# tbennun/capital

Measured on NVIDIA H100. Metric: cholesky_tflops_fp64, higher is better.
Workload: dtype f64

## Files before the change

### capital_b200/csrc/leaf.cu

```cuda
#include "common.cuh"
#include "tile64.cuh"
#include <cooperative_groups.h>
#include <cfloat>
#include <stdlib.h>
#include <type_traits>
namespace cg = cooperative_groups;

namespace {
constexpr int LD = LEAF_MAX + 1;

__device__ __forceinline__ double fast_rsqrt(double d) {
  if (!(d > 1e-30 && d < 1e30)) return rsqrt(d);
  double y = (double)rsqrtf((float)d);
  const double h = 0.5 * d;
  y = y * fma(-h, y * y, 1.5);
  y = y * fma(-h, y * y, 1.5);
  return y;
}

__device__ void leaf_factor_invert(int nb, double* __restrict__ a, double* __restrict__ r, double* __restrict__ t, int* info,
                                   int pivot_base) {
  const int tid = threadIdx.x, tx = tid & 15, ty = tid >> 4;
  for (int k = 0; k < nb; k++) {
    if (tid < 64 && tid >= k && tid < nb) {
      double d = a[k + k * LD];
      if (!(d > 0.0)) {
        if (tid == k) atomicCAS(info, 0, pivot_base + k + 1);
        d = 1.0;
      }
      const double rs = rsqrt(d);
      r[k + tid * LD] = (tid == k) ? d * rs : a[k + tid * LD] * rs;
    }
    __syncthreads();
#pragma unroll
    for (int ia = 0; ia < 4; ia++) {
      const int i = ty + 16 * ia;
      if (i > k && i < nb) {
        const double ri = r[k + i * LD];
#pragma unroll
        for (int jb = 0; jb < 4; jb++) {
          const int j = tx + 16 * jb;
          if (j >= i && j < nb) a[i + j * LD] -= ri * r[k + j * LD];
        }
      }
    }
    __syncthreads();
  }
#pragma unroll
  for (int ia = 0; ia < 4; ia++) {
    const int i = ty + 16 * ia;
#pragma unroll
    for (int jb = 0; jb < 4; jb++) {
      const int j = tx + 16 * jb;
      if (i < nb && j < nb) {
        if (i > j) r[i + j * LD] = 0.0;
        a[i + j * LD] = (i == j) ? 1.0 / r[i + i * LD] : 0.0;
      }
    }
  }
  __syncthreads();
  int lg = 0;
  for (int bs = 1; bs < nb; bs <<= 1, lg++) {
    const int span = 2 * bs;
    const int npairs = (nb + span - 1) / span;
    const int per = bs * bs, total = npairs * per;
    for (int idx = tid; idx < total; idx += 256) {
      const int p = idx >> (2 * lg), e = idx & (per - 1);
      const int li = e & (bs - 1), lj = e >> lg;
      const int o = p * span, i = o + li, j = o + bs + lj;
      if (j < nb) {
        double s = 0.0;
        const int kend = o + bs;
        for (int k = i; k < kend; k++) s += a[i + k * LD] * r[k + j * LD];
        t[i + j * LD] = s;
      }
    }
    __syncthreads();
    for (int idx = tid; idx < total; idx += 256) {
      const int p = idx >> (2 * lg), e = idx & (per - 1);
      const int li = e & (bs - 1), lj = e >> lg;
      const int o = p * span, i = o + li, j = o + bs + lj;
      if (j < nb) {
        double s = 0.0;
        for (int k = o + bs; k <= j; k++) s += t[i + k * LD] * a[k + j * LD];
        a[i + j * LD] = -s;
      }
    }
    __syncthreads();
  }
}

__device__ __forceinline__ void leaf_load(int nb, const double* W, long long ldw, double* __restrict__ a) {
  for (int idx = threadIdx.x; idx < nb * nb; idx += 256) {
    const int i = idx % nb, j = idx / nb;
    a[i + j * LD] = (i <= j) ? __ldcg(W + i + (long long)j * ldw) : 0.0;
  }
}
__device__ __forceinline__ void leaf_store(int nb, const double* a, const double* r, double* __restrict__ R,
                                           long long ldr, double* __restrict__ Ri, long long ldri, double* __restrict__ RiT,
                                           long long ldrit) {
  for (int idx = threadIdx.x; idx < nb * nb; idx += 256) {
    const int i = idx % nb, j = idx / nb;
    R[i + (long long)j * ldr] = r[i + j * LD];
    Ri[i + (long long)j * ldri] = a[i + j * LD];
  }
  if (RiT != nullptr) {
    for (int idx = threadIdx.x; idx < nb * nb; idx += 256) {
      const int j = idx % nb, i = idx / nb;
      RiT[j + (long long)i * ldrit] = a[i + j * LD];
    }
  }
}

__global__ void __launch_bounds__(256, 1)
    leaf_kernel(int nb, const double* W, long long ldw, double* __restrict__ R, long long ldr, double* __restrict__ Ri,
                long long ldri, double* __restrict__ RiT, long long ldrit, int* __restrict__ info, BatchStrides bs,
                int pivot_base) {
  extern __shared__ double sm[];
  double* a = sm;
  double* r = sm + LEAF_MAX * LD;
  double* t = sm + 2 * LEAF_MAX * LD;
  const long long b = blockIdx.x;
  W += b * bs.w; R += b * bs.r; Ri += b * bs.ri; info += b;
  if (RiT != nullptr) RiT += b * bs.rit;
  leaf_load(nb, W, ldw, a);
  __syncthreads();
  leaf_factor_invert(nb, a, r, t, info, pivot_base);
  leaf_store(nb, a, r, R, ldr, Ri, ldri, RiT, ldrit);
}

template <bool ACCUM>
__device__ __forceinline__ void tile_store(double* __restrict__ dst, long long ld, const double* sC) {
  const int r2 = (threadIdx.x & 31) * 2, c0 = threadIdx.x >> 5;
#pragma unroll
  for (int r = 0; r < 8; r++) {
    const int c = c0 + 8 * r;
    double2 v = *reinterpret_cast<const double2*>(sC + c * TLD + r2);
    double2* p = reinterpret_cast<double2*>(dst + r2 + (long long)c * ld);
    if (ACCUM) { const double2 o = __ldcg(p); v.x += o.x; v.y += o.y; }
    *p = v;
  }
}
__device__ __forceinline__ void tile_store_from_rowmajor(double* __restrict__ dst, long long ld, const double* sCr) {
  const int c2 = (threadIdx.x & 31) * 2, r0 = threadIdx.x >> 5;
#pragma unroll
  for (int r = 0; r < 8; r++) {
    const int row = r0 + 8 * r;
    const double2 v = *reinterpret_cast<const double2*>(sCr + row * TLD + c2);
    *reinterpret_cast<double2*>(dst + c2 + (long long)row * ld) = v;
  }
}

__device__ __forceinline__ double shfl_d(double v, int src) { return __shfl_sync(0xffffffffu, v, src); }

template <int I, int END, int STEP = 1, typename F>
__device__ __forceinline__ void static_for(F&& f) {
  if constexpr (I < END) {
    f(std::integral_constant<int, I>{});
    static_for<I + STEP, END, STEP>(f);
  }
}

__device__ __forceinline__ void warp_potrf_trtri_32(double (&c)[32], double* __restrict__ sRb, double* __restrict__ sXb, double* __restrict__ sXTb,
                                                    double* __restrict__ ub, int lane, int* info, int pivot_base, long long* dbg2) {
  double myrs = 0.0;
  if (dbg2 && lane == 0) dbg2[0] = clock64();
  double dl = 0.0;
  static_for<0, 32>([&](auto ic) { constexpr int i = decltype(ic)::value; if (lane == i) dl = c[i]; });
  const bool equil = !__all_sync(0xffffffffu, dl >= 0x1p-400 && dl <= 0x1p400);
  double fl = 1.0;
  if (equil) {
    if (dl > 0.0 && dl <= DBL_MAX) fl = ldexp(1.0, -(ilogb(dl) >> 1));
    static_for<0, 32>([&](auto ic) { constexpr int i = decltype(ic)::value; c[i] = c[i] * shfl_d(fl, i) * fl; });
  }
  double a = shfl_d(c[0], 0), l = shfl_d(c[0], 1), b = shfl_d(c[1], 1);
  static_for<0, 32, 2>([&](auto kc) {
    constexpr int k = decltype(kc)::value;
    if (!(a > 0.0)) { if (lane == k) atomicCAS(info, 0, pivot_base + k + 1); a = 1.0; }
    double det = fma(b, a, -(l * l));
    if (!(det > 0.0)) { if (lane == k + 1) atomicCAS(info, 0, pivot_base + k + 2); det = 1.0; }
    const double ra = fast_rsqrt(a), rdet = fast_rsqrt(det);
    const double sa = a * ra, lk = l * ra, rs2 = sa * rdet;
    const double u0 = (lane > k) ? c[k] * ra : (lane == k ? sa : 0.0);
    const double t1 = fma(-lk, u0, c[k + 1]);
    const double u1 = (lane > k + 1) ? t1 * rs2 : (lane == k + 1 ? det * rdet * ra : 0.0);
    c[k] = u0;
    c[k + 1] = u1;
    if (lane == k) myrs = ra;
    if (lane == k + 1) myrs = rs2;
    double* row0 = ub + (k & 2) * 32;
    double* row1 = row0 + 32;
    row0[lane] = u0;
    row1[lane] = u1;
    __syncwarp();
    if constexpr (k + 2 < 32) {
      c[k + 2] = fma(-row1[k + 2], u1, fma(-row0[k + 2], u0, c[k + 2]));
      c[k + 3] = fma(-row1[k + 3], u1, fma(-row0[k + 3], u0, c[k + 3]));
      a = shfl_d(c[k + 2], k + 2);
      l = shfl_d(c[k + 2], k + 3);
      b = shfl_d(c[k + 3], k + 3);
      static_for<k + 4, 32>([&](auto ic) {
        constexpr int i = decltype(ic)::value;
        c[i] = fma(-row1[i], u1, fma(-row0[i], u0, c[i]));
      });
    }
  });
  if (equil) {
    const double gl = 1.0 / fl;
    static_for<0, 32>([&](auto ic) { constexpr int i = decltype(ic)::value; c[i] *= gl; });
    myrs *= fl;
  }
  if (dbg2 && lane == 0) dbg2[1] = clock64();
#pragma unroll
  for (int i = 0; i < 32; i++) sRb[lane * TLD + i] = c[i];
  __syncwarp();
  const int g16 = lane >> 4, jl = lane & 15, base = 16 * g16;
  double xl[16];
  static_for<0, 16>([&](auto rc_) { constexpr int r = decltype(rc_)::value; xl[r] = (r == jl) ? myrs : 0.0; });
  static_for<0, 15>([&](auto sc) {
    constexpr int il = 14 - decltype(sc)::value;
    const double rsi = shfl_d(myrs, base + il);
    double s0 = 0.0, s1 = 0.0, s2 = 0.0, s3 = 0.0;
    static_for<il + 1, 16>([&](auto tc) {
      constexpr int t = decltype(tc)::value;
      const double rit = sRb[(base + t) * TLD + base + il];
      if constexpr ((t & 3) == 0) s0 = fma(rit, xl[t], s0);
      else if constexpr ((t & 3) == 1) s1 = fma(rit, xl[t], s1);
      else if constexpr ((t & 3) == 2) s2 = fma(rit, xl[t], s2);
      else s3 = fma(rit, xl[t], s3);
    });
    if (jl > il) xl[il] = -rsi * ((s0 + s1) + (s2 + s3));
  });
  double* xs = ub + 128;
  double* ts = ub + 128 + 512;
  static_for<0, 16>([&](auto rc_) {
    constexpr int r = decltype(rc_)::value;
    xs[lane * 16 + r] = xl[r];
    sXb[lane * TLD + base + r] = xl[r];
    sXTb[(base + r) * TLD + lane] = xl[r];
  });
  __syncwarp();
  {
    double rc[16], tr[8];
    static_for<0, 16>([&](auto tc) { constexpr int t = decltype(tc)::value; rc[t] = sRb[(16 + jl) * TLD + t]; });
    static_for<0, 8>([&](auto rr) {
      constexpr int r = decltype(rr)::value;
      const int i = 8 * g16 + r;
      double s = 0.0;
      static_for<0, 16>([&](auto tc) {
        constexpr int t = decltype(tc)::value;
        s = fma(xs[t * 16 + i], rc[t], s);
      });
      tr[r] = s;
      ts[jl * 16 + i] = s;
    });
    __syncwarp();
    double xc[16];
    static_for<0, 16>([&](auto tc) { constexpr int t = decltype(tc)::value; xc[t] = xs[(16 + jl) * 16 + t]; });
    static_for<0, 8>([&](auto rr) {
      constexpr int r = decltype(rr)::value;
      const int i = 8 * g16 + r;
      double s = 0.0;
      static_for<0, 16>([&](auto tc) {
        constexpr int t = decltype(tc)::value;
        s = fma(ts[t * 16 + i], xc[t], s);
      });
      sXb[(16 + jl) * TLD + i] = -s;
      sXTb[i * TLD + 16 + jl] = -s;
    });
    (void)tr;
  }
  __syncwarp();
  if (dbg2 && lane == 0) dbg2[2] = clock64();
}

__device__ __forceinline__ void mma32(double (&acc)[2][2], const double* As, int ar, const double* Bs, int bc, int k0) {
  const int lane = threadIdx.x & 31, w = threadIdx.x >> 5, g = lane >> 2, q = lane & 3;
  const double* ap = As + (ar + (w & 3) * 8 + g) * TLD + k0 + q;
  const double* bp = Bs + (bc + (w >> 2) * 16 + g) * TLD + k0 + q;
#pragma unroll
  for (int k = 0; k < 32; k += 4) {
    const double a = ap[k], b0 = bp[k], b1 = bp[8 * TLD + k];
    dmma884(acc[0][0], acc[0][1], a, b0);
    dmma884(acc[1][0], acc[1][1], a, b1);
  }
}
#define M32_ROW ((w & 3) * 8 + g)
#define M32_COL(j, e) ((w >> 2) * 16 + (j) * 8 + 2 * q + (e))

__device__ void leaf64_fast(double* __restrict__ sA, double* __restrict__ sR, double* __restrict__ sX, double* __restrict__ sXT,
                            double* __restrict__ ub, int* info, int pivot_base, long long* dbg2 = nullptr) {
  const int tid = threadIdx.x, lane = tid & 31, w = tid >> 5, g = lane >> 2, q = lane & 3;
  for (int idx = tid; idx < 64 * 64; idx += 256) {
    const int r = idx & 63, cidx = idx >> 6;
    sR[cidx * TLD + r] = 0.0; sX[cidx * TLD + r] = 0.0; sXT[cidx * TLD + r] = 0.0;
  }
  __syncthreads();
  double c[32];
#pragma unroll 1
  for (int half = 0; half < 2; half++) {
    const int o = half * 32;
    if (half == 1) {
      double acc[2][2] = {{0.0, 0.0}, {0.0, 0.0}};
      mma32(acc, sX, 0, sA, 32, 0);
#pragma unroll
      for (int j = 0; j < 2; j++)
#pragma unroll
        for (int e = 0; e < 2; e++) sR[(32 + M32_COL(j, e)) * TLD + M32_ROW] = acc[j][e];
      __syncthreads();
      double acc2[2][2] = {{0.0, 0.0}, {0.0, 0.0}};
      mma32(acc2, sR + 32 * TLD, 0, sR + 32 * TLD, 0, 0);
#pragma unroll
      for (int j = 0; j < 2; j++)
#pragma unroll
        for (int e = 0; e < 2; e++) sA[(32 + M32_COL(j, e)) * TLD + 32 + M32_ROW] -= acc2[j][e];
      __syncthreads();
    }
    if (w == 0) {
#pragma unroll
      for (int i = 0; i < 32; i++) c[i] = sA[(o + lane) * TLD + o + i];
      warp_potrf_trtri_32(c, sR + o * TLD + o, sX + o * TLD + o, sXT + o * TLD + o, ub, lane, info, pivot_base + o,
                          (dbg2 && half == 0) ? dbg2 : nullptr);
      if (dbg2 && half == 0 && lane == 0) dbg2[3] = clock64();
    }
    __syncthreads();
  }
  {
    double acc[2][2] = {{0.0, 0.0}, {0.0, 0.0}};
    mma32(acc, sXT, 0, sR, 32, 0);
    __syncthreads();
#pragma unroll
    for (int j = 0; j < 2; j++)
#pragma unroll
      for (int e = 0; e < 2; e++) sA[M32_ROW * TLD + 32 + M32_COL(j, e)] = acc[j][e];
    __syncthreads();
    double acc2[2][2] = {{0.0, 0.0}, {0.0, 0.0}};
    mma32(acc2, sA, 0, sX, 32, 32);
#pragma unroll
    for (int j = 0; j < 2; j++)
#pragma unroll
      for (int e = 0; e < 2; e++) {
        const double v = -acc2[j][e];
        sX[(32 + M32_COL(j, e)) * TLD + M32_ROW] = v;
        sXT[M32_ROW * TLD + 32 + M32_COL(j, e)] = v;
      }
  }
  __syncthreads();
}

template <int CW>
__global__ void __cluster_dims__(CW, 1, 1) __launch_bounds__(256, 1)
    basecase_kernel(int nb, double* __restrict__ W, long long ldw, double* __restrict__ R, long long ldr, double* __restrict__ Ri,
                    long long ldri, double* __restrict__ RiT, long long ldrit, int* __restrict__ info, long long* __restrict__ dbg,
                    BatchStrides bstr, int pivot_base) {
  {
    const long long b = blockIdx.y;
    W += b * bstr.w; R += b * bstr.r; Ri += b * bstr.ri; RiT += b * bstr.rit; info += b;
  }
  extern __shared__ __align__(16) double sm[];
  double* sA = sm;
  double* sB = sm + TILE_DOUBLES;
  double* sT = sm + 2 * TILE_DOUBLES;
  cg::cluster_group cluster = cg::this_cluster();
  const int rank = (int)cluster.block_rank();
  const int T = nb >> 6;
  double acc[4][2][2];
  int dbgi = 0;
#define DBG_STAMP() do { if (dbg && rank == 0 && threadIdx.x == 0) dbg[dbgi++] = clock64(); } while (0)
  DBG_STAMP();

  double* sU = sm + 3 * TILE_DOUBLES;
  auto do_leaf = [&](int jb) {
    const long long o = (long long)jb * 64;
    __syncthreads();
    tile_load(sA, W + o + o * ldw, ldw);
    __syncthreads();
    if (dbg && jb == 0 && threadIdx.x == 0) dbg[20] = clock64();
    leaf64_fast(sA, sB, sT, sU, sm + 4 * TILE_DOUBLES, info, pivot_base + jb * 64, (dbg && jb == 0) ? dbg + 24 : nullptr);
    if (dbg && jb == 0 && threadIdx.x == 0) dbg[21] = clock64();
    tile_store<false>(R + o + o * ldr, ldr, sB);
    tile_store<false>(Ri + o + o * ldri, ldri, sT);
    tile_store<false>(RiT + o + o * ldrit, ldrit, sU);
    __syncthreads();
  };
  auto do_trailing = [&](int jb, int i, int j) {
    const long long o = (long long)jb * 64;
    __syncthreads();
    tile_load(sA, R + o + (long long)i * 64 * ldr, ldr);
    tile_load(sB, R + o + (long long)j * 64 * ldr, ldr);
    __syncthreads();
    acc_zero(acc);
    tile_mma(acc, sA, sB);
    acc_to_smem_colmajor(acc, sT, -1.0);
    __syncthreads();
    tile_store<true>(W + (long long)i * 64 + (long long)j * 64 * ldw, ldw, sT);
  };

  if (rank == 0) do_leaf(0);
  DBG_STAMP();
  __threadfence();
  cluster.sync();
  DBG_STAMP();
  for (int jb = 0; jb < T; jb++) {
    const long long o = (long long)jb * 64;
    int work = 0;
    for (int j = jb + 1; j < T; j++, work++) {
      if (work % CW != rank) continue;
      __syncthreads();
      tile_load(sA, Ri + o + o * ldri, ldri);
      tile_load(sB, W + o + (long long)j * 64 * ldw, ldw);
      __syncthreads();
      acc_zero(acc);
      tile_mma(acc, sA, sB);
      acc_to_smem_colmajor(acc, sT, 1.0);
      __syncthreads();
      tile_store<false>(R + o + (long long)j * 64 * ldr, ldr, sT);
    }
    if (jb == 0) DBG_STAMP();
    __threadfence();
    cluster.sync();
    if (jb == 0) DBG_STAMP();
    if (jb + 1 < T) {
      const int leaf_rank = (jb + 1) % CW;
      if (rank == leaf_rank) {
        do_trailing(jb, jb + 1, jb + 1);
        __threadfence_block();
        do_leaf(jb + 1);
      } else {
        const int slot = rank > leaf_rank ? rank - 1 : rank;
        work = 0;
        for (int j = jb + 1; j < T; j++)
          for (int i = jb + 1; i <= j; i++) {
            if (i == jb + 1 && j == jb + 1) continue;
            if (work++ % (CW - 1) != slot) continue;
            do_trailing(jb, i, j);
          }
      }
    }
    if (jb == 0) DBG_STAMP();
    __threadfence();
    cluster.sync();
    if (jb == 0) DBG_STAMP();
  }
  DBG_STAMP();
  {
    int work = 0;
    for (int j = 0; j < T; j++)
      for (int i = j + 1; i < T; i++, work++) {
        if (work % CW != rank) continue;
        for (int idx = threadIdx.x; idx < 4096; idx += 256)
          R[(long long)i * 64 + (idx & 63) + ((long long)j * 64 + (idx >> 6)) * ldr] = 0.0;
      }
  }
  for (int bs = 1; bs < T; bs <<= 1) {
    const int span = 2 * bs;
    int work = 0;
    for (int o = 0; o + bs < T; o += span) {
      const int jend = min(o + span, T);
      for (int j = o + bs; j < jend; j++)
        for (int i = o; i < o + bs; i++, work++) {
          if (work % CW != rank) continue;
          acc_zero(acc);
          for (int k = i; k < o + bs; k++) {
            __syncthreads();
            tile_load(sA, RiT + (long long)k * 64 + (long long)i * 64 * ldrit, ldrit);
            tile_load(sB, R + (long long)k * 64 + (long long)j * 64 * ldr, ldr);
            __syncthreads();
            tile_mma(acc, sA, sB);
          }
          __syncthreads();
          acc_to_smem_rowmajor(acc, sT, 1.0);
          __syncthreads();
          tile_store_from_rowmajor(W + (long long)j * 64 + (long long)i * 64 * ldw, ldw, sT);
        }
    }
    __threadfence();
    cluster.sync();
    work = 0;
    for (int o = 0; o + bs < T; o += span) {
      const int jend = min(o + span, T);
      for (int j = o + bs; j < jend; j++)
        for (int i = o; i < o + bs; i++, work++) {
          if (work % CW != rank) continue;
          acc_zero(acc);
          for (int k = o + bs; k <= j; k++) {
            __syncthreads();
            tile_load(sA, W + (long long)k * 64 + (long long)i * 64 * ldw, ldw);
            tile_load(sB, Ri + (long long)k * 64 + (long long)j * 64 * ldri, ldri);
            __syncthreads();
            tile_mma(acc, sA, sB);
          }
          __syncthreads();
          acc_to_smem_colmajor(acc, sA, -1.0);
          acc_to_smem_rowmajor(acc, sB, -1.0);
          __syncthreads();
          tile_store<false>(Ri + (long long)i * 64 + (long long)j * 64 * ldri, ldri, sA);
          tile_store_from_rowmajor(RiT + (long long)j * 64 + (long long)i * 64 * ldrit, ldrit, sB);
        }
    }
    __threadfence();
    cluster.sync();
  }
  DBG_STAMP();
}
}

namespace {
constexpr int LEAF_SMEM = 3 * LEAF_MAX * LD * (int)sizeof(double);
constexpr int BASECASE_SMEM = (4 * TILE_DOUBLES + 128 + 512 + 256) * (int)sizeof(double);
}
capital_status_t leaf_init(capital_ctx* ctx) {
  CAP_CUDA(cudaFuncSetAttribute(leaf_kernel, cudaFuncAttributeMaxDynamicSharedMemorySize, LEAF_SMEM));
  CAP_CUDA(cudaFuncSetAttribute(basecase_kernel<2>, cudaFuncAttributeMaxDynamicSharedMemorySize, BASECASE_SMEM));
  CAP_CUDA(cudaFuncSetAttribute(basecase_kernel<4>, cudaFuncAttributeMaxDynamicSharedMemorySize, BASECASE_SMEM));
  CAP_CUDA(cudaFuncSetAttribute(basecase_kernel<8>, cudaFuncAttributeMaxDynamicSharedMemorySize, BASECASE_SMEM));
  return CAPITAL_OK;
}

capital_status_t leaf_cholinv(capital_ctx* ctx, cudaStream_t st, int nb, const double* W, int64_t ldw, double* R, int64_t ldr, double* Ri,
                              int64_t ldri, double* RiT, int64_t ldrit, const LeafBatch* bt, int pivot_base) {
  if (nb <= 0) return CAPITAL_OK;
  if (nb > LEAF_MAX || (bt && (bt->batch < 1 || bt->batch > INT32_MAX))) return CAPITAL_ERR_INVALID;
  constexpr int smem = LEAF_SMEM;
  const int tli = ctx->tl_begin(st, 4, nb);
  leaf_kernel<<<bt ? (unsigned)bt->batch : 1u, 256, smem, st>>>(nb, W, ldw, R, ldr, Ri, ldri, RiT, ldrit, bt ? bt->info : ctx->d_info,
                                                                bt ? bt->s : BatchStrides{}, pivot_base);
  ctx->tl_end(st, tli);
  ctx->counters.kernel_launches++;
  ctx->counters.leaf_launches++;
  CAP_CUDA(cudaGetLastError());
  return CAPITAL_OK;
}

capital_status_t basecase_cholinv(capital_ctx* ctx, cudaStream_t st, int nb, double* W, int64_t ldw, double* R, int64_t ldr, double* Ri,
                                  int64_t ldri, double* RiT, int64_t ldrit, const LeafBatch* bt, int pivot_base) {
  if (nb % 64 != 0 || nb < 64 || nb > BASECASE_MAX || RiT == nullptr) return CAPITAL_ERR_INVALID;
  const int cw = bt ? bt->cw : 8;
  if (bt && (bt->batch < 1 || bt->batch > 65535)) return CAPITAL_ERR_INVALID;
  auto kernel = cw == 2 ? basecase_kernel<2> : cw == 4 ? basecase_kernel<4> : cw == 8 ? basecase_kernel<8> : nullptr;
  if (!kernel) return CAPITAL_ERR_INVALID;
  constexpr int smem = BASECASE_SMEM;
  long long* dbg = nullptr;
  if (getenv("CAPITAL_BC_DEBUG") && !bt) {
    CAP_TRY(ctx->workspace("bc_dbg", 64 * sizeof(long long), (void**)&dbg));
    CAP_CUDA(cudaMemsetAsync(dbg, 0, 64 * sizeof(long long), st));
  }
  const int tli = ctx->tl_begin(st, 3, nb);
  kernel<<<dim3(cw, bt ? (unsigned)bt->batch : 1u), 256, smem, st>>>(nb, W, ldw, R, ldr, Ri, ldri, RiT, ldrit, bt ? bt->info : ctx->d_info,
                                                                      dbg, bt ? bt->s : BatchStrides{}, pivot_base);
  ctx->tl_end(st, tli);
  if (dbg) {
    long long h[32];
    CAP_CUDA(cudaMemcpyAsync(h, dbg, sizeof(h), cudaMemcpyDeviceToHost, st));
    CAP_CUDA(cudaStreamSynchronize(st));
    fprintf(stderr, "[bc nb=%d] leaf0=%lld bar=%lld panel0=%lld bar=%lld trail0+leaf1=%lld bar=%lld | chol_total=%lld inverse=%lld total=%lld cycles\n", nb,
            h[1] - h[0], h[2] - h[1], h[3] - h[2], h[4] - h[3], h[5] - h[4], h[6] - h[5], h[7] - h[0], h[8] - h[7], h[8] - h[0]);
    fprintf(stderr, "   leaf64: load=%lld total=%lld | warp32: pre=%lld potrf=%lld trtri=%lld store=%lld\n", h[20] - h[0], h[21] - h[20], h[24] - h[20],
            h[25] - h[24], h[26] - h[25], h[27] - h[26]);
  }
  ctx->counters.kernel_launches++;
  ctx->counters.leaf_launches++;
  CAP_CUDA(cudaGetLastError());
  return CAPITAL_OK;
}
```

### capital_b200/csrc/tile64.cuh

```cuda
#pragma once
#include "common.cuh"

namespace {
constexpr int TLD = 68;
constexpr int TILE_DOUBLES = 64 * TLD;

__device__ __forceinline__ void dmma884(double& c0, double& c1, double a, double b) {
  asm("mma.sync.aligned.m8n8k4.row.col.f64.f64.f64.f64 {%0,%1}, {%2}, {%3}, {%0,%1};" : "+d"(c0), "+d"(c1) : "d"(a), "d"(b));
}
__device__ __forceinline__ void tile_load(double* __restrict__ dst, const double* src, long long ld) {
  const int k2 = (threadIdx.x & 31) * 2, c0 = threadIdx.x >> 5;
  double2 v[8];
#pragma unroll
  for (int r = 0; r < 8; r++) v[r] = __ldcg(reinterpret_cast<const double2*>(src + k2 + (long long)(c0 + 8 * r) * ld));
#pragma unroll
  for (int r = 0; r < 8; r++) *reinterpret_cast<double2*>(dst + (c0 + 8 * r) * TLD + k2) = v[r];
}
__device__ __forceinline__ void tile_mma(double (&acc)[4][2][2], const double* As, const double* Bs) {
  const int lane = threadIdx.x & 31, w = threadIdx.x >> 5, g = lane >> 2, q = lane & 3;
  const double* ap = As + ((w & 1) * 32 + g) * TLD + q;
  const double* bp = Bs + ((w >> 1) * 16 + g) * TLD + q;
#pragma unroll 4
  for (int k0 = 0; k0 < 64; k0 += 4) {
    double af[4], bf[2];
#pragma unroll
    for (int i = 0; i < 4; i++) af[i] = ap[i * 8 * TLD + k0];
#pragma unroll
    for (int j = 0; j < 2; j++) bf[j] = bp[j * 8 * TLD + k0];
#pragma unroll
    for (int i = 0; i < 4; i++)
#pragma unroll
      for (int j = 0; j < 2; j++) dmma884(acc[i][j][0], acc[i][j][1], af[i], bf[j]);
  }
}
__device__ __forceinline__ void acc_zero(double (&acc)[4][2][2]) {
#pragma unroll
  for (int i = 0; i < 4; i++)
#pragma unroll
    for (int j = 0; j < 2; j++) acc[i][j][0] = acc[i][j][1] = 0.0;
}
#define TILE_ROW(i) ((w & 1) * 32 + (i) * 8 + g)
#define TILE_COL(j, e) ((w >> 1) * 16 + (j) * 8 + 2 * q + (e))
__device__ __forceinline__ void acc_to_smem_colmajor(const double (&acc)[4][2][2], double* __restrict__ sC, double scale) {
  const int lane = threadIdx.x & 31, w = threadIdx.x >> 5, g = lane >> 2, q = lane & 3;
#pragma unroll
  for (int i = 0; i < 4; i++)
#pragma unroll
    for (int j = 0; j < 2; j++)
#pragma unroll
      for (int e = 0; e < 2; e++) sC[TILE_COL(j, e) * TLD + TILE_ROW(i)] = scale * acc[i][j][e];
}
__device__ __forceinline__ void acc_to_smem_rowmajor(const double (&acc)[4][2][2], double* __restrict__ sC, double scale) {
  const int lane = threadIdx.x & 31, w = threadIdx.x >> 5, g = lane >> 2, q = lane & 3;
#pragma unroll
  for (int i = 0; i < 4; i++)
#pragma unroll
    for (int j = 0; j < 2; j++)
#pragma unroll
      for (int e = 0; e < 2; e++) sC[TILE_ROW(i) * TLD + TILE_COL(j, e)] = scale * acc[i][j][e];
}
}
```

Measured before the change: 33.46.

## Pipeline cluster basecase with split arrive/wait barriers and overlapped inversion

Restructures the clustered basecase kernel so rank 0 runs the critical-path leaf factorizations while the other ranks handle panels, trailing updates and triangular-inverse tiles. Full cluster.sync calls are replaced by split barrier.cluster arrive/wait, and leaf input is kept resident in shared memory. A precomputed schedule lets inverse tiles run early, interleaved with the factorization. K-loops in the inverse use double-buffered cp.async. This is meant to cut barrier stalls and serialization on the leaf critical path, at the cost of much more complex scheduling and a greater risk of ordering bugs.

```diff
diff --git a/capital_b200/csrc/leaf.cu b/capital_b200/csrc/leaf.cu
--- a/capital_b200/csrc/leaf.cu
+++ b/capital_b200/csrc/leaf.cu
@@ -348,6 +348,13 @@
   __syncthreads();
 }
 
+__device__ __forceinline__ void cluster_arrive() { asm volatile("barrier.cluster.arrive.release.aligned;" ::: "memory"); }
+__device__ __forceinline__ void cluster_wait() { asm volatile("barrier.cluster.wait.acquire.aligned;" ::: "memory"); }
+__device__ __forceinline__ void cluster_publish() {
+  __threadfence();
+  cluster_arrive();
+}
+
 template <int CW>
 __global__ void __cluster_dims__(CW, 1, 1) __launch_bounds__(256, 1)
     basecase_kernel(int nb, double* __restrict__ W, long long ldw, double* __restrict__ R, long long ldr, double* __restrict__ Ri,
@@ -361,27 +368,33 @@
   double* sA = sm;
   double* sB = sm + TILE_DOUBLES;
   double* sT = sm + 2 * TILE_DOUBLES;
-  cg::cluster_group cluster = cg::this_cluster();
-  const int rank = (int)cluster.block_rank();
+  double* sU = sm + 3 * TILE_DOUBLES;
+  double* ub = sm + 4 * TILE_DOUBLES;
+  const int rank = (int)cg::this_cluster().block_rank();
   const int T = nb >> 6;
   double acc[4][2][2];
-  int dbgi = 0;
-#define DBG_STAMP() do { if (dbg && rank == 0 && threadIdx.x == 0) dbg[dbgi++] = clock64(); } while (0)
-  DBG_STAMP();
-
-  double* sU = sm + 3 * TILE_DOUBLES;
+#define DBG_STAMP(r, i) do { if (dbg && rank == (r) && threadIdx.x == 0) dbg[i] = clock64(); } while (0)
+  DBG_STAMP(0, 0);
+
   auto do_leaf = [&](int jb) {
     const long long o = (long long)jb * 64;
-    __syncthreads();
-    tile_load(sA, W + o + o * ldw, ldw);
-    __syncthreads();
     if (dbg && jb == 0 && threadIdx.x == 0) dbg[20] = clock64();
-    leaf64_fast(sA, sB, sT, sU, sm + 4 * TILE_DOUBLES, info, pivot_base + jb * 64, (dbg && jb == 0) ? dbg + 24 : nullptr);
+    leaf64_fast(sA, sB, sT, sU, ub, info, pivot_base + jb * 64, (dbg && jb == 0) ? dbg + 24 : nullptr);
     if (dbg && jb == 0 && threadIdx.x == 0) dbg[21] = clock64();
     tile_store<false>(R + o + o * ldr, ldr, sB);
     tile_store<false>(Ri + o + o * ldri, ldri, sT);
     tile_store<false>(RiT + o + o * ldrit, ldrit, sU);
-    __syncthreads();
+  };
+  auto do_panel = [&](int jb, int j, const double* As) {
+    const long long o = (long long)jb * 64;
+    __syncthreads();
+    tile_load(sB, W + o + (long long)j * 64 * ldw, ldw);
+    __syncthreads();
+    acc_zero(acc);
+    tile_mma(acc, As, sB);
+    acc_to_smem_colmajor(acc, sT, 1.0);
+    __syncthreads();
+    tile_store<false>(R + o + (long long)j * 64 * ldr, ldr, sT);
   };
   auto do_trailing = [&](int jb, int i, int j) {
     const long long o = (long long)jb * 64;
@@ -396,53 +409,145 @@
     tile_store<true>(W + (long long)i * 64 + (long long)j * 64 * ldw, ldw, sT);
   };
 
-  if (rank == 0) do_leaf(0);
-  DBG_STAMP();
-  __threadfence();
-  cluster.sync();
-  DBG_STAMP();
-  for (int jb = 0; jb < T; jb++) {
-    const long long o = (long long)jb * 64;
-    int work = 0;
-    for (int j = jb + 1; j < T; j++, work++) {
-      if (work % CW != rank) continue;
+  auto kloop = [&](int kb, int ke, const double* Ap, long long lda, const double* Bp, long long ldb) {
+    __syncthreads();
+    tile_load_async(sA, Ap + (long long)kb * 64, lda);
+    tile_load_async(sB, Bp + (long long)kb * 64, ldb);
+    cp_async_commit();
+    for (int k = kb; k < ke; k++) {
+      const bool odd = (k - kb) & 1;
+      if (k + 1 < ke) {
+        tile_load_async(odd ? sA : sT, Ap + (long long)(k + 1) * 64, lda);
+        tile_load_async(odd ? sB : sU, Bp + (long long)(k + 1) * 64, ldb);
+        cp_async_commit();
+        cp_async_wait<1>();
+      } else {
+        cp_async_wait<0>();
+      }
       __syncthreads();
-      tile_load(sA, Ri + o + o * ldri, ldri);
-      tile_load(sB, W + o + (long long)j * 64 * ldw, ldw);
+      tile_mma(acc, odd ? sT : sA, odd ? sU : sB);
       __syncthreads();
-      acc_zero(acc);
-      tile_mma(acc, sA, sB);
-      acc_to_smem_colmajor(acc, sT, 1.0);
-      __syncthreads();
-      tile_store<false>(R + o + (long long)j * 64 * ldr, ldr, sT);
-    }
-    if (jb == 0) DBG_STAMP();
-    __threadfence();
-    cluster.sync();
-    if (jb == 0) DBG_STAMP();
-    if (jb + 1 < T) {
-      const int leaf_rank = (jb + 1) % CW;
-      if (rank == leaf_rank) {
-        do_trailing(jb, jb + 1, jb + 1);
-        __threadfence_block();
-        do_leaf(jb + 1);
+    }
+  };
+  auto inv_phase1 = [&](int o, int bs, int i, int j) {
+    acc_zero(acc);
+    kloop(i, o + bs, RiT + (long long)i * 64 * ldrit, ldrit, R + (long long)j * 64 * ldr, ldr);
+    acc_to_smem_rowmajor(acc, sT, 1.0);
+    __syncthreads();
+    tile_store_from_rowmajor(W + (long long)j * 64 + (long long)i * 64 * ldw, ldw, sT);
+  };
+  auto inv_phase2 = [&](int o, int bs, int i, int j) {
+    acc_zero(acc);
+    kloop(o + bs, j + 1, W + (long long)i * 64 * ldw, ldw, Ri + (long long)j * 64 * ldri, ldri);
+    acc_to_smem_colmajor(acc, sA, -1.0);
+    acc_to_smem_rowmajor(acc, sB, -1.0);
+    __syncthreads();
+    tile_store<false>(Ri + (long long)i * 64 + (long long)j * 64 * ldri, ldri, sA);
+    tile_store_from_rowmajor(RiT + (long long)j * 64 + (long long)i * 64 * ldrit, ldrit, sB);
+  };
+  constexpr int INV_POST = 64, INV_NEVER = 1000;
+  int* isched = reinterpret_cast<int*>(ub + 896);
+  auto inv_step = [&](int v) { return (v >> 1) <= T - 2 ? (v >> 1) : INV_POST; };
+  auto inv_vis = [&](int s) { return s == INV_POST ? INV_NEVER : 2 * s + 2; };
+  if (threadIdx.x == 0) {
+    int* vis = isched + 24;
+    for (int o = 0; o < T; o++) vis[o] = 2 * o;
+    for (int lvl = 0, bs = 1; bs < T; bs <<= 1, lvl++)
+      for (int p = 0, o = 0; o + bs < T; o += 2 * bs, p++) {
+        const int s1 = inv_step(max(vis[o], 2 * (o + bs) - 1));
+        const int s2 = inv_step(max(inv_vis(s1), vis[o + bs]));
+        isched[8 * lvl + 2 * p] = s1;
+        isched[8 * lvl + 2 * p + 1] = s2;
+        vis[o] = max(max(vis[o], vis[o + bs]), inv_vis(s2));
+      }
+  }
+  __syncthreads();
+  auto inv_tiles = [&](auto&& pick, auto&& f) {
+    for (int c = 4; c >= 1; c--)
+      for (int lvl = 0, bs = 1; bs < T; bs <<= 1, lvl++) {
+        if (c > bs) continue;
+        for (int p = 0, o = 0; o + bs < T; o += 2 * bs, p++) {
+          if (pick(8 * lvl + 2 * p)) {
+            const int i = o + bs - c;
+            for (int j = o + bs; j < min(o + 2 * bs, T); j++) f(bs, 0, o, i, j);
+          }
+          if (pick(8 * lvl + 2 * p + 1)) {
+            const int j = o + bs + c - 1;
+            if (j < T)
+              for (int i = o; i < o + bs; i++) f(bs, 1, o, i, j);
+          }
+        }
+      }
+  };
+  auto inv_tile = [&](int bs, int ph, int o, int i, int j) {
+    if (ph == 0) inv_phase1(o, bs, i, j);
+    else inv_phase2(o, bs, i, j);
+  };
+
+  for (int jb = -1; jb + 1 < T; jb++) {
+    const long long o = (long long)jb * 64, o1 = o + 64;
+    if (rank == 0) {
+      if (jb < 0) {
+        tile_load(sA, W, ldw);
+        __syncthreads();
       } else {
-        const int slot = rank > leaf_rank ? rank - 1 : rank;
-        work = 0;
-        for (int j = jb + 1; j < T; j++)
-          for (int i = jb + 1; i <= j; i++) {
-            if (i == jb + 1 && j == jb + 1) continue;
-            if (work++ % (CW - 1) != slot) continue;
-            do_trailing(jb, i, j);
-          }
-      }
-    }
-    if (jb == 0) DBG_STAMP();
-    __threadfence();
-    cluster.sync();
-    if (jb == 0) DBG_STAMP();
-  }
-  DBG_STAMP();
+        __syncthreads();
+        tile_load(sU, W + o + o1 * ldw, ldw);
+        tile_load(sA, W + o1 + o1 * ldw, ldw);
+        __syncthreads();
+        acc_zero(acc);
+        tile_mma(acc, sT, sU);
+        acc_to_smem_colmajor(acc, sB, 1.0);
+        __syncthreads();
+        tile_store<false>(R + o + o1 * ldr, ldr, sB);
+        if (jb == 0) DBG_STAMP(0, 3);
+        acc_zero(acc);
+        tile_mma(acc, sB, sB);
+        acc_add_to_smem_colmajor(acc, sA, -1.0);
+        cluster_publish();
+        __syncthreads();
+        if (jb == 0) DBG_STAMP(0, 4);
+      }
+      do_leaf(jb + 1);
+      if (jb == 0) DBG_STAMP(0, 5);
+      if (jb >= 0) cluster_wait();
+      if (jb == 0) DBG_STAMP(0, 6);
+    } else if (jb >= 0) {
+      const int slot = rank - 1;
+      if (slot < T - jb - 2) {
+        __syncthreads();
+        tile_load(sA, Ri + o + o * ldri, ldri);
+      }
+      int work = 0;
+      for (int j = jb + 2; j < T; j++)
+        if (work++ % (CW - 1) == slot) do_panel(jb, j, sA);
+      if (jb == 0) DBG_STAMP(1, 11);
+      cluster_publish();
+      cluster_wait();
+      if (jb == 0) DBG_STAMP(1, 12);
+      work = 0;
+      for (int j = jb + 1; j < T; j++)
+        for (int i = jb + 1; i <= j; i++) {
+          if (i == jb + 1 && j == jb + 1) continue;
+          if (work++ % (CW - 1) != slot) continue;
+          do_trailing(jb, i, j);
+        }
+      work = 0;
+      inv_tiles([&](int g) { return isched[g] == jb; }, [&](int bs, int ph, int oo, int i, int j) {
+        const int r = work % (CW - 1), round = work / (CW - 1);
+        work++;
+        if (((round & 1) ? r : CW - 2 - r) == slot) inv_tile(bs, ph, oo, i, j);
+      });
+      if (jb == 0) DBG_STAMP(1, 13);
+    }
+    if (jb < 0) DBG_STAMP(0, 1);
+    cluster_publish();
+    cluster_wait();
+    if (jb < 0) { DBG_STAMP(0, 2); DBG_STAMP(1, 10); }
+    if (jb == 0) DBG_STAMP(0, 9);
+  }
+  DBG_STAMP(0, 7);
+  DBG_STAMP(1, 14);
   {
     int work = 0;
     for (int j = 0; j < T; j++)
@@ -452,62 +557,28 @@
           R[(long long)i * 64 + (idx & 63) + ((long long)j * 64 + (idx >> 6)) * ldr] = 0.0;
       }
   }
-  for (int bs = 1; bs < T; bs <<= 1) {
-    const int span = 2 * bs;
-    int work = 0;
-    for (int o = 0; o + bs < T; o += span) {
-      const int jend = min(o + span, T);
-      for (int j = o + bs; j < jend; j++)
-        for (int i = o; i < o + bs; i++, work++) {
-          if (work % CW != rank) continue;
-          acc_zero(acc);
-          for (int k = i; k < o + bs; k++) {
-            __syncthreads();
-            tile_load(sA, RiT + (long long)k * 64 + (long long)i * 64 * ldrit, ldrit);
-            tile_load(sB, R + (long long)k * 64 + (long long)j * 64 * ldr, ldr);
-            __syncthreads();
-            tile_mma(acc, sA, sB);
-          }
-          __syncthreads();
-          acc_to_smem_rowmajor(acc, sT, 1.0);
-          __syncthreads();
-          tile_store_from_rowmajor(W + (long long)j * 64 + (long long)i * 64 * ldw, ldw, sT);
-        }
-    }
-    __threadfence();
-    cluster.sync();
-    work = 0;
-    for (int o = 0; o + bs < T; o += span) {
-      const int jend = min(o + span, T);
-      for (int j = o + bs; j < jend; j++)
-        for (int i = o; i < o + bs; i++, work++) {
-          if (work % CW != rank) continue;
-          acc_zero(acc);
-          for (int k = o + bs; k <= j; k++) {
-            __syncthreads();
-            tile_load(sA, W + (long long)k * 64 + (long long)i * 64 * ldw, ldw);
-            tile_load(sB, Ri + (long long)k * 64 + (long long)j * 64 * ldri, ldri);
-            __syncthreads();
-            tile_mma(acc, sA, sB);
-          }
-          __syncthreads();
-          acc_to_smem_colmajor(acc, sA, -1.0);
-          acc_to_smem_rowmajor(acc, sB, -1.0);
-          __syncthreads();
-          tile_store<false>(Ri + (long long)i * 64 + (long long)j * 64 * ldri, ldri, sA);
-          tile_store_from_rowmajor(RiT + (long long)j * 64 + (long long)i * 64 * ldrit, ldrit, sB);
-        }
-    }
-    __threadfence();
-    cluster.sync();
-  }
-  DBG_STAMP();
+  auto owner = [&](int w) { const int r = w % CW; return ((w / CW) & 1) ? CW - 1 - r : r; };
+  for (int lvl = 0, bs = 1; bs < T; bs <<= 1, lvl++)
+    for (int ph = 0; ph < 2; ph++) {
+      bool any = false;
+      for (int p = 0, o = 0; o + bs < T; o += 2 * bs, p++) any |= isched[8 * lvl + 2 * p + ph] == INV_POST;
+      if (!any) continue;
+      int work = 0;
+      inv_tiles([&](int g) { return (g >> 3) == lvl && (g & 1) == ph && isched[g] == INV_POST; },
+                [&](int bs_, int ph_, int oo, int i, int j) {
+                  if (owner(work++) == rank) inv_tile(bs_, ph_, oo, i, j);
+                });
+      cluster_publish();
+      cluster_wait();
+    }
+  DBG_STAMP(0, 8);
+#undef DBG_STAMP
 }
 }
 
 namespace {
 constexpr int LEAF_SMEM = 3 * LEAF_MAX * LD * (int)sizeof(double);
-constexpr int BASECASE_SMEM = (4 * TILE_DOUBLES + 128 + 512 + 256) * (int)sizeof(double);
+constexpr int BASECASE_SMEM = (4 * TILE_DOUBLES + 128 + 512 + 256) * (int)sizeof(double) + 32 * (int)sizeof(int);
 }
 capital_status_t leaf_init(capital_ctx* ctx) {
   CAP_CUDA(cudaFuncSetAttribute(leaf_kernel, cudaFuncAttributeMaxDynamicSharedMemorySize, LEAF_SMEM));
@@ -553,9 +624,12 @@
     long long h[32];
     CAP_CUDA(cudaMemcpyAsync(h, dbg, sizeof(h), cudaMemcpyDeviceToHost, st));
     CAP_CUDA(cudaStreamSynchronize(st));
-    fprintf(stderr, "[bc nb=%d] leaf0=%lld bar=%lld panel0=%lld bar=%lld trail0+leaf1=%lld bar=%lld | chol_total=%lld inverse=%lld total=%lld cycles\n", nb,
-            h[1] - h[0], h[2] - h[1], h[3] - h[2], h[4] - h[3], h[5] - h[4], h[6] - h[5], h[7] - h[0], h[8] - h[7], h[8] - h[0]);
-    fprintf(stderr, "   leaf64: load=%lld total=%lld | warp32: pre=%lld potrf=%lld trtri=%lld store=%lld\n", h[20] - h[0], h[21] - h[20], h[24] - h[20],
+    fprintf(stderr, "[bc nb=%d] rank 0: leaf0=%lld barA0=%lld panel(0,1)=%lld trail(1,1)=%lld leaf1=%lld barB0=%lld barA1=%lld | chol_total=%lld "
+                    "inverse=%lld total=%lld cycles\n", nb, h[1] - h[0], h[2] - h[1], h[3] - h[2], h[4] - h[3], h[5] - h[4], h[6] - h[5],
+            h[9] - h[6], h[7] - h[0], h[8] - h[7], h[8] - h[0]);
+    fprintf(stderr, "   rank 1: panel0=%lld barB0=%lld trail0=%lld to_chol_end=%lld\n", h[11] - h[10], h[12] - h[11], h[13] - h[12],
+            h[14] - h[13]);
+    fprintf(stderr, "   leaf64: total=%lld | warp32: pre=%lld potrf=%lld trtri=%lld store=%lld\n", h[21] - h[20], h[24] - h[20],
             h[25] - h[24], h[26] - h[25], h[27] - h[26]);
   }
   ctx->counters.kernel_launches++;
diff --git a/capital_b200/csrc/tile64.cuh b/capital_b200/csrc/tile64.cuh
--- a/capital_b200/csrc/tile64.cuh
+++ b/capital_b200/csrc/tile64.cuh
@@ -59,4 +59,28 @@
 #pragma unroll
       for (int e = 0; e < 2; e++) sC[TILE_ROW(i) * TLD + TILE_COL(j, e)] = scale * acc[i][j][e];
 }
+__device__ __forceinline__ void acc_add_to_smem_colmajor(const double (&acc)[4][2][2], double* __restrict__ sC, double scale) {
+  const int lane = threadIdx.x & 31, w = threadIdx.x >> 5, g = lane >> 2, q = lane & 3;
+#pragma unroll
+  for (int i = 0; i < 4; i++)
+#pragma unroll
+    for (int j = 0; j < 2; j++)
+#pragma unroll
+      for (int e = 0; e < 2; e++) {
+        double* p = sC + TILE_COL(j, e) * TLD + TILE_ROW(i);
+        const double v = scale * acc[i][j][e];
+        *p = v + *p;
+      }
 }
+__device__ __forceinline__ void tile_load_async(double* __restrict__ dst, const double* src, long long ld) {
+  const int k2 = (threadIdx.x & 31) * 2, c0 = threadIdx.x >> 5;
+#pragma unroll
+  for (int r = 0; r < 8; r++) {
+    const unsigned d = (unsigned)__cvta_generic_to_shared(dst + (c0 + 8 * r) * TLD + k2);
+    asm volatile("cp.async.cg.shared.global [%0], [%1], 16;" ::"r"(d), "l"(src + k2 + (long long)(c0 + 8 * r) * ld) : "memory");
+  }
+}
+__device__ __forceinline__ void cp_async_commit() { asm volatile("cp.async.commit_group;" ::: "memory"); }
+template <int N>
+__device__ __forceinline__ void cp_async_wait() { asm volatile("cp.async.wait_group %0;" ::"n"(N) : "memory"); }
+}
```

Result: faster. 34.12 (median of 6 runs) (+2.0%).
